# AutomationLabs-sh/AutomationLabsModelPredictiveControl.jl

Measured on AMD Instinct MI355X. Metric: MPC steps/s (batch=4096, nx=12, nu=4, N=30), higher is better.
Workload: dtype f64; 1 GPU; configs[1]: hover-linearised quadrotor nx=12 nu=4 N=30, 4096 instances per GPU, shared model, x0 amplitude classes 0.3/1.0/3.0 interleaved, cold start every step; batch_per_gpu=4096, global_batch=4096, seed=0x5eed0002, setup_ramp_steps=300, admm_max_iter=6, check_every=6, polish=1, warm_state_kept=False, parallelism=instances sharded over 1 GPU(s), 16-instance tile per workgroup

## Files before the change

### automationlabsmodelpredictivecontrol.jl_amd/_capi.py

```python
from __future__ import annotations

import ctypes
import os

import numpy as np

_HERE = os.path.dirname(os.path.abspath(__file__))
LIB_PATH = os.environ.get("ALMPC_LIB") or os.path.join(_HERE, "lib", "libalmpc.so")

ALMPC_OK = 0
ERR_NAMES = {0: "ALMPC_OK", -1: "ALMPC_ERR_INVALID", -2: "ALMPC_ERR_NO_DEVICE", -3: "ALMPC_ERR_HIP",
             -4: "ALMPC_ERR_UNSUPPORTED", -5: "ALMPC_ERR_NOT_DESIGNED", -6: "ALMPC_ERR_NUMERIC"}
FLAG_TIMING = 0x1
FLAG_STRUCTURED = 0x2
SOLVED, MAX_ITER, NON_FINITE, INFEASIBLE = 0, 1, 2, 3


class AlmpcError(RuntimeError):
    def __init__(self, code, msg=""):
        self.code = code
        super().__init__(f"{ERR_NAMES.get(code, code)}: {msg}")


class almpc_opts(ctypes.Structure):
# ... 175 lines not shown
    L.almpc_group_sqp_fnn_state_multipliers.argtypes = [_hp, _dp]
    L.almpc_group_sqp_fnn_solve.argtypes = [_hp, ctypes.c_int, ctypes.c_double, ctypes.POINTER(almpc_opts), _ip, _ip, _dp]
    L.almpc_group_x0_staging.argtypes = [_hp, ctypes.POINTER(_dp)]
    L.almpc_group_update_initialization_staged.argtypes = [_hp, ctypes.POINTER(_dp)]
    L.almpc_group_get_results_async.argtypes = [_hp, ctypes.c_uint32]
    L.almpc_group_get_results_wait.argtypes = [_hp, ctypes.c_int, _dp, _dp, _dp, _dp, _dp, _ip, _ip, _ip]
    for nm_ in ("almpc_group_set_terminal_equality", "almpc_group_set_rho_profile", "almpc_group_set_structured_fallback", "almpc_group_set_state_box",
                "almpc_group_design_batched", "almpc_group_relin_fnn_setup", "almpc_group_relin_fnn_step", "almpc_group_relin_fnn_step_async",
                "almpc_group_relin_fnn_advance", "almpc_group_advance_plant", "almpc_group_sqp_fnn_set_structured", "almpc_group_sqp_fnn_set_step_rule",
                "almpc_group_sqp_fnn_setup", "almpc_group_relin_densenet_setup", "almpc_group_sqp_densenet_setup", "almpc_group_sqp_fnn_start", "almpc_group_sqp_fnn_iterate", "almpc_group_sqp_fnn_skipped", "almpc_group_sqp_fnn_solve", "almpc_group_sqp_fnn_set_hessian",
                "almpc_group_sqp_fnn_set_row_multipliers", "almpc_group_sqp_fnn_state_multipliers",
                "almpc_group_x0_staging", "almpc_group_update_initialization_staged", "almpc_group_get_results_async", "almpc_group_get_results_wait"):
        getattr(L, nm_).restype = ctypes.c_int
    L.almpc_set_start_from.argtypes = [_hp, _hp]
    L.almpc_set_start_from.restype = ctypes.c_int
    L.almpc_timing_samples.argtypes = [_hp, ctypes.c_int, ctypes.POINTER(ctypes.c_int), _fp, _fp, _fp, _fp]
    L.almpc_timing_samples.restype = ctypes.c_int
    for name in ("almpc_x0_staging", "almpc_update_initialization_async", "almpc_get_results_async", "almpc_get_results_wait", "almpc_host_results",
                 "almpc_get_first_input", "almpc_group_create", "almpc_group_size", "almpc_group_shard", "almpc_group_design_shared",
                 "almpc_group_set_reference", "almpc_group_update_initialization", "almpc_group_calculate",
                 "almpc_group_calculate_async", "almpc_group_synchronize", "almpc_group_get_results"):
        getattr(L, name).restype = ctypes.c_int
    for name in ("almpc_create", "almpc_design_shared", "almpc_set_reference", "almpc_update_initialization",
                 "almpc_update_initialization_device", "almpc_calculate", "almpc_calculate_async", "almpc_synchronize",
                 "almpc_get_results", "almpc_get_design", "almpc_device_results", "almpc_get_timing", "almpc_timing_reset",
                 "almpc_timing_summary"):
        getattr(L, name).restype = ctypes.c_int
    _lib = L
    return L


OPT_NO_WARM_STATE = 0x1
OPT_FULL_FIRST_PRODUCT = 0x2
WANT = {"x": 0x01, "e_x": 0x02, "u": 0x04, "e_u": 0x08, "status": 0x10, "iters": 0x20, "polish_iters": 0x40, "u0": 0x80}
SENS = {"K0": 0x1, "dU": 0x2, "dX": 0x4}


def _sens_mask(want):
    mask = 0
    for k in ((want,) if isinstance(want, str) else want):
        if k not in SENS:
            raise ValueError(f"unknown sensitivity {k!r} (one of {sorted(SENS)})")
        mask |= SENS[k]
    if not mask:
        raise ValueError("sensitivity: nothing asked for")
    return mask


def _sens_read(get, handle, check, want, b, n, m, N):
    mask = _sens_mask(want)
    K0 = np.empty((b, n, m)) if mask & SENS["K0"] else None
    dU = np.empty((b, n, N, m)) if mask & SENS["dU"] else None
    dX = np.empty((b, n, N + 1, n)) if mask & SENS["dX"] else None
    rows = np.empty(b, dtype=np.int32)
    check(get(handle, _ptr(K0), _ptr(dU), _ptr(dX), rows.ctypes.data_as(_ip)))
    out = {"rows": rows}
    if K0 is not None: out["K0"] = K0.transpose(0, 2, 1)
    if dU is not None: out["dU"] = dU.transpose(0, 3, 2, 1)
    if dX is not None: out["dX"] = dX.transpose(0, 3, 2, 1)
    return out


def _sens_vjp(call, handle, check, g_u, g_x, act_tol, b, n, m, N):
    g_u = np.ascontiguousarray(np.asarray(g_u, dtype=np.float64).reshape(b, m, N).transpose(0, 2, 1))
    if g_x is not None:
        g_x = np.ascontiguousarray(np.asarray(g_x, dtype=np.float64).reshape(b, n, N + 1).transpose(0, 2, 1))
# ... 924 lines not shown
```

### automationlabsmodelpredictivecontrol.jl_amd/csrc/almpc_api.hip

```cpp
#include "almpc_kernels.hip.h"
#include "almpc_design.hip.h"
#include "almpc_polish_gen.hip.h"
#include "almpc_fnn.hip.h"
#include "almpc_instance.hip.h"
#include "almpc_sqp.hip.h"
#include "almpc_comm.hip.h"
#include "almpc_riccati.hip.h"
#include "almpc_sdual.hip.h"
#include "almpc_dare.hip.h"
#include "almpc_c2d.hip.h"
#include "almpc_sens.hip.h"
#include "almpc_host_math.h"
#include "almpc_switches.h"
#include "almpc_devbuf.h"
#include "../../include/almpc.h"

#ifndef ALMPC_UNITY
#define ALMPC_KERNEL_INSTANCE(...) extern template __global__ __VA_ARGS__;
#include "instances/sdual_a.inc"
#include "instances/sdual_b.inc"
#include "instances/sdual_c.inc"
#include "instances/polish_gen.inc"
#include "instances/step.inc"
#include "instances/instance.inc"
// ... 2255 lines not shown
    HIP_TRY(h, h->dOverflow.once((size_t)h->batch * 33 + 2));
    HIP_TRY(h, hipMemsetAsync(h->dOverflow, 0, 2 * sizeof(int32_t), h->stream));
    HIP_TRY(h, h->dOvfSinv.once((size_t)h->batch * (32 * 32 + 32)));
    gp.ovf = h->dOverflow; gp.ovf_ws = h->dOverflow + 2 + h->batch; gp.ovf_sinv = h->dOvfSinv;
    if (s.lazy_redo) { gp.unsolved = h->redo.dUnsolved; gp.redo_gate = h->redo.dGate; gp.step_serial = h->redo.step_serial; }
    if (h->fallback && !h->ltv && h->sd.ready && !h->sd.sqp && !h->sw.no_redo_start) {
        HIP_TRY(h, h->sd.start_ws.once((size_t)h->batch * 64));
        gp.redo_ws = h->sd.start_ws; gp.redo_sp = h->sd.NT + h->sd.MC; gp.redo_nt = h->sd.NT;
        h->sd.start_ws_fresh = true;
    }
    if (h->s0_basis_ok && !h->batched && !h->ltv && h->fS_stride == 0) gp.s0_basis = h->dS0Basis;
    if (s.mode.rows.mu && sq) { gp.rows = s.mode.rows; gp.rows_map = h->dRowMap; }
    switch (h->np_pairs) {
        case 1: HIP_TRY(h, launch_polish_gen<1>(h, gp)); break;
        case 2: HIP_TRY(h, launch_polish_gen<2>(h, gp)); break;
        case 3: HIP_TRY(h, launch_polish_gen<3>(h, gp)); break;
        default: HIP_TRY(h, launch_polish_gen<4>(h, gp)); break;
    }
    HIP_TRY(h, s.t.mark(2));
    return ALMPC_OK;
}

template <int KS>
hipError_t launch_step_fused(const AdmmParams& ap, const PolishParams& pp, size_t lds, hipStream_t st) {
    const hipError_t e = ensure_dyn_lds(reinterpret_cast<const void*>(k_step_fused<8, KS>), lds);
    if (e != hipSuccess) return e;
    hipLaunchKernelGGL((k_step_fused<8, KS>), dim3(pp.ntiles), dim3(512), lds, st, ap, pp);
    return hipGetLastError();
}

int step_fused_shared(Step& s, const PolishLayout& L) {
    almpc_handle* h = s.h;
    const AdmmParams ap = admm_params(h, s.o, s.keep_state);
    const PolishParams pp = polish_params(s, L);
    HIP_TRY(h, s.t.mark(1));
    HIP_TRY(h, h->ks == 30 ? launch_step_fused<30>(ap, pp, L.l_step, h->stream) : launch_step_fused<32>(ap, pp, L.l_step, h->stream));
    HIP_TRY(h, s.t.mark(2));
    return ALMPC_OK;
}

template <int NZC>
hipError_t launch_step_inst_wave_t(const almpc_handle* h, const AdmmInstParams& ip, const PolishParams& pp, size_t lds) {
    const hipError_t e = ensure_dyn_lds(reinterpret_cast<const void*>(k_step_inst_wave<NZC>), lds);
    if (e != hipSuccess) return e;
    hipLaunchKernelGGL((k_step_inst_wave<NZC>), dim3((unsigned)h->batch), dim3(64), lds, h->stream, ip, pp);
    return hipGetLastError();
}

int step_wave(Step& s, const PolishLayout& L, bool shared) {
    almpc_handle* h = s.h;
    if (shared) HIP_TRY(h, s.t.start());
    const AdmmInstParams ip = admm_inst_params(h, s.o, shared);
    PolishParams pp = polish_params(s, L);
    if (shared) { pp.yflags = nullptr; pp.yflag_words = 0; }
    const size_t wave = (size_t)L.per_wave + (shared ? 0 : (size_t)h->nz * h->nzs);
    const size_t lds = ((size_t)L.SL.total + wave) * sizeof(double);
    pp.sg_off = -1; pp.g_off = shared ? 0 : L.per_wave;
    pp.lds_per_wave = (int)wave;
    pp.direct = 1;
    HIP_TRY(h, s.t.mark(1));
    if (h->nzs <= 16) HIP_TRY(h, launch_step_inst_wave_t<16>(h, ip, pp, lds));
    else if (h->nzs <= 32) HIP_TRY(h, launch_step_inst_wave_t<32>(h, ip, pp, lds));
    else if (h->nzs <= 48) HIP_TRY(h, launch_step_inst_wave_t<48>(h, ip, pp, lds));
    else HIP_TRY(h, launch_step_inst_wave_t<64>(h, ip, pp, lds));
    HIP_TRY(h, s.t.mark(2));
    return ALMPC_OK;
}
// ... 1678 lines not shown
```

### automationlabsmodelpredictivecontrol.jl_amd/csrc/almpc_kernels.hip.h

```cpp
#pragma once
#include <hip/hip_runtime.h>
#include <stdint.h>

#include <map>
#include <mutex>
#include <utility>
#include <type_traits>

namespace almpc {

inline hipError_t ensure_dyn_lds(const void* fn, size_t bytes) {
    if (bytes <= 64 * 1024) return hipSuccess;
    static std::mutex mu;
    static std::map<std::pair<int, const void*>, size_t> cur;
    int dev = 0;
    hipError_t e = hipGetDevice(&dev);
    if (e != hipSuccess) return e;
    std::lock_guard<std::mutex> lock(mu);
    size_t& c = cur[std::make_pair(dev, fn)];
    if (c >= bytes) return hipSuccess;
    e = hipFuncSetAttribute(fn, hipFuncAttributeMaxDynamicSharedMemorySize, (int)bytes);
    if (e == hipSuccess) c = bytes;
    return e;
}
// ... 62 lines not shown
    const double* VFrag;
    const double* v0S;
    long v0S_stride;
    const double* Wp = nullptr;
    const double* rowc = nullptr;
    const double* HFrag;
    const double* FFrag;
    int ksf;
    const double* dvec;
    const double* rhovec;
    const double* umin;
    const double* umax;
    const double* uref;
    long uref_stride;
    const double* xref;
    long xref_stride;
    const double* fS;
    long fS_stride;
    const double* x0;
    double* xs;
    double* zs;
    double* ys;
    double* v0;
    int32_t* status;
    int32_t* iters;
    int32_t* piters;
    int32_t* perm;
    double rho, sigma, alpha, eps_abs, eps_rel;
    int max_iter, check_every, warm;
    int keep_state;
    uint32_t* yflags;
};

template <int NRB, int KS, typename AfterRequests>
__device__ __forceinline__ void admm_body(const AdmmParams& p, double* smem, AfterRequests after_requests) {
    constexpr int RP = 16 * NRB;
    static_assert(4 * KS <= RP, "K padding must fit the row padding");
    double* rhs0 = smem;
    double* rhs1 = smem + RP * TILE;
    double* red = smem + 2 * RP * TILE;
    double* e0s = red + NRB * 8 * TILE;

    const int wv = threadIdx.x >> 6, lane = threadIdx.x & 63;
    const int col = lane & 15, q = lane >> 4;
    const int inst = blockIdx.x * TILE + col;
    const bool valid = inst < p.batch;
    const int instc = valid ? inst : p.batch - 1;
    ALMPC_STAMP(blockIdx.x * NRB + wv, 0);

    constexpr int KSF_FAST = 4;
    const bool tabled = p.rowc != nullptr;
    const bool affine = !p.warm && tabled && p.Wp != nullptr;
    double af[KSF_FAST], aw[KSF_FAST], av[KSF_FAST];
#pragma unroll
    for (int ks = 0; ks < KSF_FAST; ++ks) {
        const bool on = ks < p.ksf;
        const size_t o = ((size_t)(wv * p.ksf + ks)) * 64 + lane;
        af[ks] = on ? p.FFrag[o] : 0.0;
        aw[ks] = (on && affine && 4 * ks + q < p.n) ? p.Wp[(size_t)(4 * ks + q) * p.nzs + wv * 16 + col] : 0.0;
        av[ks] = on ? p.VFrag[o] : 0.0;
    }
    int row[4];
    double dv[4], dinv[4], lo[4], hi[4], fs[4], rho[4], v0s[4], ws[4];
#pragma unroll
    for (int i = 0; i < 4; ++i) row[i] = wv * 16 + q + 4 * i;
    if (tabled) {
#pragma unroll
        for (int i = 0; i < 4; ++i) {
// ... 175 lines not shown
                r[0 * TILE] = m_rp; r[1 * TILE] = m_x; r[2 * TILE] = m_z; r[3 * TILE] = m_rd;
                r[4 * TILE] = m_hx; r[5 * TILE] = m_y; r[6 * TILE] = m_bad;
            }
        }
        __syncthreads();
        if (check) {
            double rp = 0, nx = 0, nzn = 0, rd = 0, nhx = 0, ny = 0, bad = 0;
#pragma unroll 4
            for (int w2 = 0; w2 < NRB; ++w2) {
                const double* r = red + w2 * 8 * TILE + col;
                rp = fmax(rp, r[0 * TILE]); nx = fmax(nx, r[1 * TILE]); nzn = fmax(nzn, r[2 * TILE]);
                rd = fmax(rd, r[3 * TILE]); nhx = fmax(nhx, r[4 * TILE]); ny = fmax(ny, r[5 * TILE]);
                bad = fmax(bad, r[6 * TILE]);
            }
            if (active) {
                const bool conv = (rp <= p.eps_abs + p.eps_rel * fmax(nx, nzn)) &&
                                  (rd <= p.eps_abs + p.eps_rel * fmax(fmax(nhx, ny), nf));
                if (bad > 0.0) { active = false; my_iters = it; my_status = 2; }
                else if (conv) { active = false; my_iters = it; my_status = 0; }
            }
            const bool any_active = __any(active);
            __syncthreads();
            if (!any_active) { double* t = cur; cur = nxt; nxt = t; break; }
        }
        double* t = cur; cur = nxt; nxt = t;
    }

    ALMPC_STAMP(blockIdx.x * NRB + wv, 2);
    if (valid && wv == 0 && q == 0) {
        p.iters[inst] = my_iters;
        p.status[inst] = my_status;
        p.piters[inst] = 0;
    }
    {
        int cntf = 0;
#pragma unroll
        for (int i = 0; i < 4; ++i) cntf += (row[i] < p.nz && yt[i] != 0.0) ? 1 : 0;
        cntf += __shfl_xor(cntf, 16);
        cntf += __shfl_xor(cntf, 32);
        if (q == 0) red[(wv * 8 + 0) * TILE + col] = (double)cntf;
    }
    __syncthreads();
    if (wv == 0 && q == 0) {
        int k0 = valid ? 0 : -1;
        if (valid)
            for (int w2 = 0; w2 < NRB; ++w2) k0 += (int)red[(w2 * 8 + 0) * TILE + col];
        red[(0 * 8 + 1) * TILE + col] = (double)k0;
        __builtin_amdgcn_fence(__ATOMIC_RELEASE, "wavefront");
        __builtin_amdgcn_wave_barrier();
        __builtin_amdgcn_fence(__ATOMIC_ACQUIRE, "wavefront");
        int rank = 0;
        for (int c2 = 0; c2 < TILE; ++c2) {
            const int ko = (int)red[(0 * 8 + 1) * TILE + c2];
            rank += (ko > k0 || (ko == k0 && c2 < col)) ? 1 : 0;
        }
        p.perm[blockIdx.x * TILE + rank] = valid ? inst : -1;
    }
    ALMPC_STAMP(blockIdx.x * NRB + wv, 3);

    constexpr int TS = RP + 2;
    static_assert(TILE * TS <= 2 * RP * TILE, "staging tile must fit the two rhs buffers");
    double* stage = smem;
    auto flush = [&](const double (&v)[4], double* dst) {
        __syncthreads();
#pragma unroll
        for (int i = 0; i < 4; ++i) stage[col * TS + row[i]] = v[i];
        __syncthreads();
        for (int e = 2 * threadIdx.x; e < TILE * RP; e += 2 * blockDim.x) {
            const int ci = e / RP, r = e % RP;
            const int ii = blockIdx.x * TILE + ci;
            if (ii < p.batch)
                *reinterpret_cast<d2v*>(dst + (size_t)ii * p.nzs + r) = *reinterpret_cast<const d2v*>(stage + ci * TS + r);
        }
    };
    const double v0r[4] = {v04[0], v04[1], v04[2], v04[3]};
    double y[4];
#pragma unroll
    for (int i = 0; i < 4; ++i) y[i] = rho[i] * yt[i];
    if (p.keep_state) {
        flush(x, p.xs);
        flush(y, p.ys);
    } else {
        uint32_t mk = 0;
#pragma unroll
        for (int i = 0; i < 4; ++i) {
            const uint32_t b = (uint32_t)(q + 4 * i);
            mk |= (yt[i] < 0.0 ? 1u : 0u) << b;
            mk |= (yt[i] > 0.0 ? 1u : 0u) << (16u + b);
        }
        mk |= (uint32_t)__shfl_xor((int)mk, 16);
        mk |= (uint32_t)__shfl_xor((int)mk, 32);
        if (q == 0 && valid) p.yflags[(size_t)inst * NRB + wv] = mk;
    }
    flush(z, p.zs);
    flush(v0r, p.v0);
    ALMPC_STAMP(blockIdx.x * NRB + wv, 4);
}

template <int NRB, int KS>
__global__ __launch_bounds__(64 * NRB) void k_admm(AdmmParams p) {
    extern __shared__ __attribute__((aligned(16))) double smem[];
    admm_body<NRB, KS>(p, smem, []() {});
}

struct RolloutParams {
    int n, m, N, batch, nzs;
    const double* A;
    const double* B;
    long A_stride = 0, B_stride = 0, d_stride = 0;
    const double* dvec;
    const double* w;
    const double* x0;
    const double* xref;
    long xref_stride;
    const double* uref;
    long uref_stride;
    const double* umin;
    const double* umax;
    double* x;
    double* ex;
    double* u;
    double* eu;
};

struct PolishParams {
    int nz, m, batch, nzs;
    const double* G;
    const double* dvec;
    const double* umin;
    const double* umax;
    const double* uref;
    long uref_stride;
    const double* zs;
    const double* ys;
    const uint32_t* yflags;
    int yflag_words;
    const double* v0;
    double* w;
    int32_t* status;
    int32_t* piters;
    double* sglobal;
    const int32_t* start_rows = nullptr;
    const int32_t* perm;
    int ntiles;
    int lds_per_wave;
    long G_stride, d_stride, A_stride, B_stride;
    int wave_const_off;
    int sg_off;
    int sg_shared_off;
    int g_off;
    int max_iter;
    const int* dflag = nullptr;
    int* unsolved = nullptr;
    int* redo_gate = nullptr;
    int step_serial = 0;
    int direct = 0;
    int fuse_rollout;
    int roll_g, roll_cpl;
    const double* rollM;
    int roll_s, roll_nb;
    RolloutParams roll;
};

__device__ __forceinline__ double readlane_d(double v, int l) {
    int lo = __builtin_amdgcn_readlane(__double2loint(v), l);
    int hi = __builtin_amdgcn_readlane(__double2hiint(v), l);
    return __hiloint2double(hi, lo);
}

__device__ __forceinline__ double fast_rcp_d(double v) {
    double r = __builtin_amdgcn_rcp(v);
    r = __builtin_fma(__builtin_fma(-v, r, 1.0), r, r);
    r = __builtin_fma(__builtin_fma(-v, r, 1.0), r, r);
    return r;
}

typedef double gj16_row[16];
template <int JJ>
__device__ __forceinline__ void gj16_pivot(gj16_row& r, const double (&pj)[16], const double col, const double d, const bool own, const int k,
                                           const int lane) {
    const double invd = fast_rcp_d(d);
    const bool piv = lane == k;
    const double f = piv ? -invd : col * invd;
    const double keep = piv ? 0.0 : 1.0;
#pragma unroll
    for (int jj = 0; jj < 16; ++jj) r[jj] = __builtin_fma(-f, pj[jj], keep * r[jj]);
    if (own) r[JJ] = f;
}

// ... 182 lines not shown
        prev = ev;
        src0 = (s - 1) * n;
        upart(b + 1, acc);
        if (xref_lds) asm volatile("" : "+v"(xr));
        if (ok) {
            gex[t] = ev;
            if (gx) gx[t] = ev + xr;
        }
    }
}

constexpr int POLISH_WAVES = 4;
#ifndef ALMPC_EXP_POLISH_WAVES
#define ALMPC_EXP_POLISH_WAVES 8
#endif
constexpr int POLISH_WAVES_GLDS = ALMPC_EXP_POLISH_WAVES;
constexpr int POLISH_LDS_MIN_PER_WAVE = 128 + 64 + 64 + 32;
struct PolishShared {
    int off_d, off_umin, off_umax, off_uref, off_ab, off_xref, total;
};
__host__ __device__ inline PolishShared polish_shared_layout(int n, int m, int N, int nz, int nzs, int fused) {
    PolishShared L;
    L.off_d = 0;
    L.off_umin = nzs;
    L.off_umax = L.off_umin + m;
    L.off_uref = L.off_umax + m;
    L.off_ab = L.off_uref + nz;
    L.off_xref = L.off_ab + ((fused && fused != 3) ? n * (n + m) : 0);
    L.total = (L.off_xref + (fused ? (N + 1) * n : 0) + 1) & ~1;
    return L;
}
constexpr int POLISH_GLB_PER_INST = 64 * 64;
constexpr int POLISH_SG_SHARED_CAP = 48;

typedef double d2 __attribute__((ext_vector_type(2)));

template <bool GLDS, bool GPRE, int KOFF, bool SGL = false, bool START = false>
__device__ __forceinline__ void polish_body(const PolishParams& p_arg, double* smem) {
    const PolishParams& p = p_arg;
    constexpr int CH = (GLDS || SGL) ? 8 : 16;
    constexpr int NWV = GLDS ? POLISH_WAVES_GLDS : (SGL ? 1 : POLISH_WAVES);
    const int wv = __builtin_amdgcn_readfirstlane(threadIdx.x >> 6), lane_k = threadIdx.x & 63;
    const int nz = p.nz, nzs = p.nzs;
    const double* Gp = p.G;
    const int gs = GLDS ? ((nz + 1) & ~1) : nzs;
    const PolishShared SL = polish_shared_layout(p.roll.n, p.m, p.roll.N, nz, nzs, p.fuse_rollout);
    double* shc = smem + (GLDS ? (size_t)nz * gs : 0);
    double* wave_lds = shc + SL.total + (size_t)wv * p.lds_per_wave;
    int* qcnt = nullptr;
    const bool uref_sh = p.uref_stride == 0, xref_sh = p.roll.xref_stride == 0;
    const bool per_inst = p.G_stride != 0;
    double* cd = shc + SL.off_d;
    double* cab = shc + SL.off_ab;
    if (per_inst) { cd = wave_lds + p.wave_const_off; cab = cd + nzs; }
    {
        constexpr int TPB = 64 * NWV;
        const int n = p.roll.n, m = p.m, N = p.roll.N;
        if (!per_inst)
            for (int t = threadIdx.x; t < nzs; t += TPB) shc[SL.off_d + t] = p.dvec[t];
        for (int t = threadIdx.x; t < m; t += TPB) { shc[SL.off_umin + t] = p.umin[t]; shc[SL.off_umax + t] = p.umax[t]; }
        if (uref_sh)
            for (int t = threadIdx.x; t < nz; t += TPB) shc[SL.off_uref + t] = p.uref[t];
        if (p.fuse_rollout) {
            if (!per_inst && p.fuse_rollout != 3) {
                for (int t = threadIdx.x; t < n * n; t += TPB) shc[SL.off_ab + t] = p.roll.A[t];
                for (int t = threadIdx.x; t < n * m; t += TPB) shc[SL.off_ab + n * n + t] = p.roll.B[t];
            }
            if (xref_sh)
                for (int t = threadIdx.x; t < (N + 1) * n; t += TPB) shc[SL.off_xref + t] = p.roll.xref[t];
        }
    }
    ALMPC_STAMP(8192 + blockIdx.x * 8 + wv, 0);
    if constexpr (GLDS && !GPRE) {
        const int hs = gs / 2;
        const bool lane_in = lane_k < hs;
        const int lq = lane_in ? lane_k : 0;
        for (int r0_ = wv; r0_ < nz; r0_ += POLISH_WAVES_GLDS * 8) {
            d2 v[8];
#pragma unroll
            for (int u = 0; u < 8; ++u) {
                const int r = r0_ + u * POLISH_WAVES_GLDS;
                v[u] = *reinterpret_cast<const d2*>(p.G + (size_t)(r < nz ? r : 0) * nzs + 2 * lq);
            }
#pragma unroll
            for (int u = 0; u < 8; ++u) {
                const int r = r0_ + u * POLISH_WAVES_GLDS;
                if (r < nz && lane_in) *reinterpret_cast<d2*>(smem + (size_t)r * gs + 2 * lq) = v[u];
            }
        }
    }
    if constexpr (GLDS) {
        qcnt = reinterpret_cast<int*>(shc + SL.total + (size_t)POLISH_WAVES_GLDS * p.lds_per_wave);
        if (threadIdx.x == 0) { qcnt[0] = POLISH_WAVES_GLDS; qcnt[1] = -1; }
        Gp = smem;
    }
    __syncthreads();
  auto process = [&](const int inst) {
    auto ka_ = __builtin_amdgcn_kernarg_segment_ptr();
    asm volatile("" : "+s"(ka_));
    const PolishParams& p = *(const PolishParams*)((const char*)ka_ + KOFF);
    int lane = lane_k;
    asm volatile("" : "+v"(lane));
    ALMPC_STAMP(inst, 8);
    if constexpr (!GLDS) {
        if (per_inst) {
            if constexpr (SGL) {
                double* gl = wave_lds + p.g_off;
                const char* src = reinterpret_cast<const char*>(GL(p.G) + (size_t)inst * p.G_stride) + lane * 16;
                if (lane < nzs / 2)
                    for (int r = 0; r < nz; ++r)
                        __builtin_amdgcn_global_load_lds((const __attribute__((address_space(1))) void*)(src + (size_t)r * nzs * 8),
                                                         (__attribute__((address_space(3))) void*)(gl + (size_t)r * nzs), 16, 0, 0);
                Gp = gl;
            } else
            Gp = GL(p.G) + (size_t)inst * p.G_stride;
            const int n_ = p.roll.n, m_ = p.m;
            for (int t = lane; t < nzs; t += 64) cd[t] = GL(p.dvec)[(size_t)inst * p.d_stride + t];
            if (p.fuse_rollout) {
                for (int t = lane; t < n_ * n_; t += 64) cab[t] = GL(p.roll.A)[(size_t)inst * p.A_stride + t];
                for (int t = lane; t < n_ * m_; t += 64) cab[n_ * n_ + t] = GL(p.roll.B)[(size_t)inst * p.B_stride + t];
            }
            if constexpr (SGL) __builtin_amdgcn_s_waitcnt(0);
            wave_fence_lds();
        }
    }
    const int st_in = GL(p.status)[inst];
    const size_t base = (size_t)inst * nzs;
    const int r0 = 2 * lane, r1 = 2 * lane + 1;
    const bool in0 = r0 < nz, in1 = r1 < nz;
    const bool inrow = r0 < nzs;
    const int rc = inrow ? r0 : 0;
    const bool skip = (st_in == 2);

    double* rowbuf = wave_lds;
    double* pbufa = rowbuf + 128;
    double* pbufb = pbufa + 64;
    int* wrow_s = reinterpret_cast<int*>(pbufb + 64);
    double* Sg;
    int cap2 = 64;
    bool own_slot = false;
    const bool sg_lds = SGL && p.sg_off >= 0;
    if (sg_lds) Sg = wave_lds + p.sg_off;
    else Sg = GL(p.sglobal) + (size_t)inst * POLISH_GLB_PER_INST;

    double lo0 = 0, hi0 = 0, lo1 = 0, hi1 = 0, v00, v01, w0 = 0, w1 = 0, y0, y1, z0, z1;
    double x0r = 0.0;
    if (p.fuse_rollout && lane < p.roll.n) x0r = GL(p.roll.x0)[(size_t)inst * p.roll.n + lane];
    {
        const d2 dv = *reinterpret_cast<const d2*>(cd + rc);
        const d2 vv = *reinterpret_cast<const d2*>(GL(p.v0) + base + rc);
        d2 yy;
        if (p.yflags) {
            const uint32_t wd = GL(p.yflags)[(size_t)inst * p.yflag_words + (rc >> 4)];
            const uint32_t b = (uint32_t)(rc & 15);
            yy[0] = (double)(int)((wd >> (16u + b)) & 1u) - (double)(int)((wd >> b) & 1u);
            yy[1] = (double)(int)((wd >> (17u + b)) & 1u) - (double)(int)((wd >> (b + 1u)) & 1u);
        } else {
            yy = *reinterpret_cast<const d2*>(GL(p.ys) + base + rc);
        }
        const d2 zz = *reinterpret_cast<const d2*>(GL(p.zs) + base + rc);
        v00 = vv[0]; v01 = vv[1]; y0 = yy[0]; y1 = yy[1]; z0 = zz[0]; z1 = zz[1];
        double urp0, urp1;
        if (uref_sh) {
            urp0 = shc[SL.off_uref + (in0 ? r0 : 0)]; urp1 = shc[SL.off_uref + (in1 ? r1 : 0)];
            asm volatile("" : "+v"(urp0), "+v"(urp1));
        } else {
            const double* ug = GL(p.uref) + (size_t)inst * p.uref_stride;
            urp0 = ug[in0 ? r0 : 0]; urp1 = ug[in1 ? r1 : 0];
        }
        if (in0) {
            const double di = 1.0 / dv[0], ur = urp0;
            lo0 = (shc[SL.off_umin + r0 % p.m] - ur) * di; hi0 = (shc[SL.off_umax + r0 % p.m] - ur) * di; w0 = fmin(fmax(z0, lo0), hi0);
        } else { v00 = 0.0; y0 = 0.0; z0 = 0.0; }
        if (in1) {
            const double di = 1.0 / dv[1], ur = urp1;
            lo1 = (shc[SL.off_umin + r1 % p.m] - ur) * di; hi1 = (shc[SL.off_umax + r1 % p.m] - ur) * di; w1 = fmin(fmax(z1, lo1), hi1);
        } else { v01 = 0.0; y1 = 0.0; z1 = 0.0; }
    }
    int wrow = 0, wsd = 0;
    double wbnd = 0.0;
    double lam = 0.0;
    bool act0 = false, act1 = false;
    double bnd0 = 0.0, bnd1 = 0.0;
    double t0 = v00, t1 = v01;
    int k = 0;
    bool overflow = false;
    ALMPC_ACC_DECL
    wrow_s[lane] = 0;
    const int hpos = lane & 31, hhf = lane >> 5;
    double Sr[16];
#pragma unroll
    for (int t = 0; t < 16; ++t) Sr[t] = 0.0;
    auto bcast16 = [&](const double* buf, double (&o)[16]) {
// ... 297 lines not shown
                if (r1 == jmin) w1 = bval;
                ALMPC_ACC(5);
                add_row(m, jmin, bval, sd);
                fresh = false;
                continue;
            }
            if (!act0) w0 = t0;
            if (!act1) w1 = t1;
            bool ok = true;
            int vi = 0;
            if (k > 0) {
                const bool mine = lowhalf && pos < k;
                const double viol = mine ? ((wsd > 0) ? -lam : lam) : -__builtin_inf();
                const double lmax = wave_max(mine ? fabs(lam) : 0.0);
                const double vmax = wave_max(viol);
                ok = vmax <= 1e-12 * fmax(1.0, lmax);
                vi = __builtin_ctzll(__ballot(mine && viol == vmax));
            }
            if (ok) {
                if (fresh) { fin = 0; return; }
                recompute(m);
                fresh = true;
                --it;
                continue;
            }
            remove_pos(m, vi);
            fresh = false;
        }
    };
    auto tier2_home = [&](int need) {
        if constexpr (GLDS) {
            if (p.sg_shared_off >= 0 && need <= POLISH_SG_SHARED_CAP) {
                int got = 0;
                if (lane == 0) got = (atomicCAS(qcnt + 1, -1, wv) == -1) ? 1 : 0;
                got = __builtin_amdgcn_readfirstlane(got);
                if (got) { own_slot = true; cap2 = POLISH_SG_SHARED_CAP; Sg = shc + p.sg_shared_off; }
            }
        }
    };
    auto slot_to_global = [&]() {
        double* Gs = GL(p.sglobal) + (size_t)inst * POLISH_GLB_PER_INST;
        for (int c = 0; c < POLISH_SG_SHARED_CAP; c += 8) {
            double v[8];
#pragma unroll
            for (int t = 0; t < 8; ++t) v[t] = Sg[(c + t) * 64 + lane];
#pragma unroll
            for (int t = 0; t < 8; ++t) Gs[(c + t) * 64 + lane] = v[t];
        }
        for (int c = POLISH_SG_SHARED_CAP; c < 64; ++c) Gs[c * 64 + lane] = (c == lane) ? 1.0 : 0.0;
        __builtin_amdgcn_fence(__ATOMIC_RELEASE, "workgroup");
        __builtin_amdgcn_wave_barrier();
        __builtin_amdgcn_fence(__ATOMIC_ACQUIRE, "workgroup");
        if (lane == 0) atomicExch(qcnt + 1, -1);
        own_slot = false; cap2 = 64; Sg = Gs;
    };
    auto to_global = [&]() {
#pragma unroll
        for (int t = 0; t < 16; ++t) {
            Sg[(16 * hhf + t) * 64 + hpos] = Sr[t];
            Sg[(16 * hhf + t) * 64 + 32 + hpos] = 0.0;
        }
#pragma unroll 4
        for (int c = 32; c < cap2; ++c) Sg[c * 64 + lane] = 0.0;
        if (lane >= 32 && lane < cap2) Sg[lane * 64 + lane] = 1.0;
        if (lane >= 32) lam = 0.0;
        sync_s(PolishMode<true>{});
    };
// ... 297 lines not shown
                const int t = t0 + 64 * u + lane;
                tt[u] = t < nx ? t : nx - 1;
                const int kq = (int)(((float)tt[u] + 0.5f) * inv_n);
                ev[u] = Z[(size_t)tt[u] + (size_t)kq * m];
            }
            if (xref_sh) {
#pragma unroll
                for (int u = 0; u < 4; ++u) xr[u] = shc[SL.off_xref + tt[u]];
                asm volatile("" : "+v"(xr[0]), "+v"(xr[1]), "+v"(xr[2]), "+v"(xr[3]));
            } else {
                const double* xg = GL(rp.xref) + (size_t)inst * rp.xref_stride;
#pragma unroll
                for (int u = 0; u < 4; ++u) xr[u] = xg[tt[u]];
            }
#pragma unroll
            for (int u = 0; u < 4; ++u) {
                const int t = t0 + 64 * u + lane;
                if (t < nx) {
                    GL(rp.ex)[xo + t] = ev[u];
                    GL(rp.x)[xo + t] = (t < n) ? x0r : ev[u] + xr[u];
                }
            }
        }
        ALMPC_STAMP(inst, 14);
    }
  };

    if constexpr (GLDS) {
        ALMPC_STAMP(8192 + blockIdx.x * 8 + wv, 1);
        [[maybe_unused]] int nproc = 0;
        for (int i = wv;;) {
            const int tile = (i >> 4) * (int)gridDim.x + (int)blockIdx.x;
            if (tile >= p.ntiles) break;
            const int inst = p.perm[tile * 16 + (i & 15)];
            if (inst >= 0) {
                process(inst);
                ++nproc;
            }
            if (lane_k == 0) i = atomicAdd(qcnt, 1);
            i = __builtin_amdgcn_readfirstlane(i);
        }
        ALMPC_STAMP(8192 + blockIdx.x * 8 + wv, 2);
#ifdef ALMPC_STAMPS
        if (g_stamps && (threadIdx.x & 63) == 0) g_stamps[(size_t)(8192 + blockIdx.x * 8 + wv) * 16 + 3] = nproc;
#endif
    } else {
        const int slot = blockIdx.x * NWV + wv;
        if (p.direct) {
            if (slot < p.batch) process(slot);
        } else if (slot < p.ntiles * 16) {
            const int inst = p.perm[(slot % p.ntiles) * 16 + slot / p.ntiles];
            if (inst >= 0) process(inst);
        }
    }
}

template <bool GLDS>
__global__ __launch_bounds__(64 * (GLDS ? POLISH_WAVES_GLDS : POLISH_WAVES))
__attribute__((amdgpu_waves_per_eu(GLDS ? POLISH_WAVES_GLDS / 4 : 2, GLDS ? POLISH_WAVES_GLDS / 4 : 2)))
void k_polish(PolishParams p_arg) {
    extern __shared__ __attribute__((aligned(16))) double smem[];
    polish_body<GLDS, false, 0>(p_arg, smem);
}

template <int START = 0>
__global__ __launch_bounds__(64) void k_polish_sgl(PolishParams p_arg) {
    extern __shared__ __attribute__((aligned(16))) double smem[];
    polish_body<false, false, 0, true, START != 0>(p_arg, smem);
}

constexpr int STEP_KOFF = (int)((sizeof(AdmmParams) + 7) & ~size_t(7));

template <int NRB, int KS>
__global__ __launch_bounds__(64 * NRB) __attribute__((amdgpu_waves_per_eu(2, 2)))
void k_step_fused(AdmmParams ap, PolishParams pp) {
    extern __shared__ __attribute__((aligned(16))) double smem[];
    if constexpr (NRB != POLISH_WAVES_GLDS) return;
    const int wv = __builtin_amdgcn_readfirstlane(threadIdx.x >> 6), lane = threadIdx.x & 63;
    const int gs = (pp.nz + 1) & ~1, hs = gs / 2;
    auto request_g = [&]() __attribute__((always_inline)) {
        for (int r = wv; r < pp.nz; r += NRB) {
            if (lane < hs) {
                const char* src = reinterpret_cast<const char*>(pp.G + (size_t)r * pp.nzs) + lane * 16;
                __builtin_amdgcn_global_load_lds((const __attribute__((address_space(1))) void*)src,
                                                 (__attribute__((address_space(3))) void*)(smem + (size_t)r * gs), 16, 0, 0);
            }
        }
    };
    admm_body<NRB, KS>(ap, smem + (size_t)pp.nz * gs, request_g);
    __builtin_amdgcn_s_waitcnt(0);
    __syncthreads();
    polish_body<true, true, STEP_KOFF>(pp, smem);
}


template <int WAVES>
__global__ __launch_bounds__(64 * WAVES) void k_rollout(RolloutParams p) {
    extern __shared__ __attribute__((aligned(16))) double smem[];
    const int n = p.n, m = p.m, N = p.N;
    const int nz = m * N, nx = n * (N + 1);
    double* As = smem;
    double* Bs = As + n * n;
    double* wbuf = Bs + n * m;
    ALMPC_STAMP(blockIdx.x * WAVES + (threadIdx.x >> 6), 4);
    const double* Ag = p.A + (size_t)blockIdx.x * WAVES * p.A_stride;
    const double* Bg = p.B + (size_t)blockIdx.x * WAVES * p.B_stride;
    for (int t = threadIdx.x; t < n * n; t += blockDim.x) As[t] = Ag[t];
    for (int t = threadIdx.x; t < n * m; t += blockDim.x) Bs[t] = Bg[t];
    __syncthreads();
    const int wv = threadIdx.x >> 6, lane = threadIdx.x & 63;
    const int inst = blockIdx.x * WAVES + wv;
    if (inst >= p.batch) return;
    ALMPC_STAMP(inst, 0);
    double* e = wbuf + (size_t)wv * (nx + nz);
    double* v = e + nx;
    for (int r = lane; r < nz; r += 64) {
        const double ur = p.uref[(size_t)inst * p.uref_stride + r];
        const double uu = fmin(fmax(p.w[(size_t)inst * p.nzs + r] * p.dvec[(size_t)inst * p.d_stride + r] + ur, p.umin[r % m]), p.umax[r % m]);
        const double ev = uu - ur;
        v[r] = ev;
        p.eu[(size_t)inst * nz + r] = ev;
        p.u[(size_t)inst * nz + r] = uu;
// ... 70 lines not shown
```

### include/almpc.h

```cpp
#ifndef ALMPC_H
#define ALMPC_H

#include <stdint.h>

#ifdef __cplusplus
extern "C" {
#endif

#define ALMPC_VERSION_MAJOR 0
#define ALMPC_VERSION_MINOR 1

typedef struct almpc_handle almpc_handle;

typedef enum almpc_status {
    ALMPC_OK = 0,
    ALMPC_ERR_INVALID = -1,
    ALMPC_ERR_NO_DEVICE = -2,
    ALMPC_ERR_HIP = -3,
    ALMPC_ERR_UNSUPPORTED = -4,
    ALMPC_ERR_NOT_DESIGNED = -5,
    ALMPC_ERR_NUMERIC = -6
} almpc_status;

typedef enum almpc_solve_status {
    ALMPC_SOLVED = 0,
    ALMPC_MAX_ITER = 1,
    ALMPC_NON_FINITE = 2,
    ALMPC_INFEASIBLE = 3
} almpc_solve_status;

typedef struct almpc_opts {
    double rho;
    double sigma;
    double alpha;
    double eps_abs;
    double eps_rel;
    int32_t max_iter;
    int32_t check_every;
    int32_t polish;
    int32_t polish_max_iter;
    int32_t warm_start;
    int32_t reserved[3];
} almpc_opts;

#define ALMPC_OPT_NO_WARM_STATE 0x1
#define ALMPC_OPT_FULL_FIRST_PRODUCT 0x2

void almpc_default_opts(almpc_opts* opts);

#define ALMPC_FLAG_TIMING 0x1u
#define ALMPC_FLAG_STRUCTURED 0x2u

int almpc_create(almpc_handle** out, int n, int m, int N, int batch, int device_id, uint32_t flags);
void almpc_destroy(almpc_handle* h);
const char* almpc_last_error(const almpc_handle* h);

int almpc_set_terminal_equality(almpc_handle* h, int on);

int almpc_set_rho_profile(almpc_handle* h, int mode);

int almpc_set_step_fusion(almpc_handle* h, int on);

int almpc_set_structured_fallback(almpc_handle* h, int on);

int almpc_set_start_from(almpc_handle* h, almpc_handle* src);

int almpc_set_state_box(almpc_handle* h, const double* xmin, const double* xmax);

int almpc_design_shared(almpc_handle* h, const double* A, const double* B, const double* Q,
                        const double* R, const double* S, const double* P, const double* umin,
                        const double* umax, const double* xmin, const double* xmax, double rho,
                        double sigma);

int almpc_design_batched(almpc_handle* h, const double* A_batch, const double* B_batch, const double* Q,
                         const double* R, const double* S, const double* P, int P_per_instance,
                         const double* umin, const double* umax, double rho, double sigma);

int almpc_design_ltv(almpc_handle* h, const double* A_all, const double* B_all, const double* c_all, const double* xbar,
                     const double* ubar, const double* xref, const double* uref, const double* Q, const double* R,
// ... 207 lines not shown
```

Baseline: 17590 batch-steps/s (one step = 4096 instance QP solves).

## Hand off ADMM state to polish through LDS records instead of HBM

In the fused step kernel, the ADMM phase now writes each instance's z, v0, sign mask, status and instance id into per-rank LDS records (wave slots plus the shared second-tier slot) and preloads polish constants. The polish phase then reads from these records instead of round-tripping through global zs/v0/yflags/status and perm. This removes HBM writes and reads between the two phases and the redundant constant reload. It adds an atomic counter so the shared slot is not claimed by a polish wave before staged records are consumed. It keeps an opt-out flag for the old HBM path.

```diff
diff --git a/automationlabsmodelpredictivecontrol.jl_amd/_capi.py b/automationlabsmodelpredictivecontrol.jl_amd/_capi.py
--- a/automationlabsmodelpredictivecontrol.jl_amd/_capi.py
+++ b/automationlabsmodelpredictivecontrol.jl_amd/_capi.py
@@ -231,6 +231,7 @@
 
 OPT_NO_WARM_STATE = 0x1
 OPT_FULL_FIRST_PRODUCT = 0x2
+OPT_HBM_HANDOFF = 0x4
 WANT = {"x": 0x01, "e_x": 0x02, "u": 0x04, "e_u": 0x08, "status": 0x10, "iters": 0x20, "polish_iters": 0x40, "u0": 0x80}
 SENS = {"K0": 0x1, "dU": 0x2, "dX": 0x4}
 
diff --git a/automationlabsmodelpredictivecontrol.jl_amd/csrc/almpc_api.hip b/automationlabsmodelpredictivecontrol.jl_amd/csrc/almpc_api.hip
--- a/automationlabsmodelpredictivecontrol.jl_amd/csrc/almpc_api.hip
+++ b/automationlabsmodelpredictivecontrol.jl_amd/csrc/almpc_api.hip
@@ -2311,7 +2311,8 @@
 int step_fused_shared(Step& s, const PolishLayout& L) {
     almpc_handle* h = s.h;
     const AdmmParams ap = admm_params(h, s.o, s.keep_state);
-    const PolishParams pp = polish_params(s, L);
+    PolishParams pp = polish_params(s, L);
+    pp.handoff = (!s.keep_state && L.sg_shared_off >= 0 && !(s.o.reserved[0] & ALMPC_OPT_HBM_HANDOFF)) ? 1 : 0;
     HIP_TRY(h, s.t.mark(1));
     HIP_TRY(h, h->ks == 30 ? launch_step_fused<30>(ap, pp, L.l_step, h->stream) : launch_step_fused<32>(ap, pp, L.l_step, h->stream));
     HIP_TRY(h, s.t.mark(2));
diff --git a/automationlabsmodelpredictivecontrol.jl_amd/csrc/almpc_kernels.hip.h b/automationlabsmodelpredictivecontrol.jl_amd/csrc/almpc_kernels.hip.h
--- a/automationlabsmodelpredictivecontrol.jl_amd/csrc/almpc_kernels.hip.h
+++ b/automationlabsmodelpredictivecontrol.jl_amd/csrc/almpc_kernels.hip.h
@@ -118,8 +118,17 @@
     uint32_t* yflags;
 };
 
-template <int NRB, int KS, typename AfterRequests>
-__device__ __forceinline__ void admm_body(const AdmmParams& p, double* smem, AfterRequests after_requests) {
+__device__ __forceinline__ void lds_barrier();
+
+constexpr int HANDOFF_STATUS = 8, HANDOFF_INST = 9;
+__device__ __forceinline__ int handoff_rot(int rank) { return 4 * (rank & 7); }
+
+struct NoHandoff {
+    static constexpr bool possible = false;
+};
+
+template <int NRB, int KS, typename AfterRequests, typename Hand>
+__device__ __forceinline__ void admm_body(const AdmmParams& p, double* smem, AfterRequests after_requests, const Hand& hand) {
     constexpr int RP = 16 * NRB;
     static_assert(4 * KS <= RP, "K padding must fit the row padding");
     double* rhs0 = smem;
@@ -361,14 +370,67 @@
         p.status[inst] = my_status;
         p.piters[inst] = 0;
     }
-    {
+    auto count_guess = [&]() {
         int cntf = 0;
 #pragma unroll
         for (int i = 0; i < 4; ++i) cntf += (row[i] < p.nz && yt[i] != 0.0) ? 1 : 0;
         cntf += __shfl_xor(cntf, 16);
         cntf += __shfl_xor(cntf, 32);
         if (q == 0) red[(wv * 8 + 0) * TILE + col] = (double)cntf;
-    }
+    };
+    auto sign_word = [&]() -> uint32_t {
+        uint32_t mk = 0;
+#pragma unroll
+        for (int i = 0; i < 4; ++i) {
+            const uint32_t b = (uint32_t)(q + 4 * i);
+            mk |= (yt[i] < 0.0 ? 1u : 0u) << b;
+            mk |= (yt[i] > 0.0 ? 1u : 0u) << (16u + b);
+        }
+        mk |= (uint32_t)__shfl_xor((int)mk, 16);
+        mk |= (uint32_t)__shfl_xor((int)mk, 32);
+        return mk;
+    };
+    if constexpr (Hand::possible) {
+        if (hand.on) {
+            static_assert(RP == 128, "a hand-off record holds 128 rows of z and of v0");
+            constexpr int TPB = 64 * NRB;
+            const double hc0 = hand.load_const((int)threadIdx.x), hc1 = hand.load_const((int)threadIdx.x + TPB);
+            count_guess();
+            lds_barrier();
+            int k0 = valid ? 0 : -1;
+            if (valid)
+                for (int w2 = 0; w2 < NRB; ++w2) k0 += (int)red[(w2 * 8 + 0) * TILE + col];
+            const int key = k0 * 16 + (15 - col);
+            int rank = 0;
+#pragma unroll
+            for (int c2 = 0; c2 < TILE; ++c2) rank += (__builtin_amdgcn_readlane(key, c2) > key) ? 1 : 0;
+            if (wv == 0 && q == 0) p.perm[blockIdx.x * TILE + rank] = valid ? inst : -1;
+            const uint32_t mk = sign_word();
+            ALMPC_STAMP(blockIdx.x * NRB + wv, 3);
+            lds_barrier();
+            double* rec = hand.record(rank);
+            const int rot = handoff_rot(rank);
+#pragma unroll
+            for (int i = 0; i < 4; ++i) {
+                const int o = (row[i] + rot) & (RP - 1);
+                rec[o] = z[i];
+                rec[RP + o] = v04[i];
+            }
+            int* ri = reinterpret_cast<int*>(rec + 2 * RP);
+            if (q == 0) ri[wv] = (int)mk;
+            if (wv == 0 && q == 0) { ri[HANDOFF_STATUS] = my_status; ri[HANDOFF_INST] = valid ? inst : -1; }
+            hand.store_const((int)threadIdx.x, hc0);
+            hand.store_const((int)threadIdx.x + TPB, hc1);
+            for (int t = (int)threadIdx.x + 2 * TPB; t < hand.SL.total; t += TPB) hand.store_const(t, hand.load_const(t));
+            if (threadIdx.x == 0) {
+                const int nvalid = p.batch - (int)blockIdx.x * TILE;
+                hand.init_queue(nvalid > NRB ? (nvalid < TILE ? nvalid : TILE) - NRB : 0);
+            }
+            ALMPC_STAMP(blockIdx.x * NRB + wv, 4);
+            return;
+        }
+    }
+    count_guess();
     __syncthreads();
     if (wv == 0 && q == 0) {
         int k0 = valid ? 0 : -1;
@@ -410,15 +472,7 @@
         flush(x, p.xs);
         flush(y, p.ys);
     } else {
-        uint32_t mk = 0;
-#pragma unroll
-        for (int i = 0; i < 4; ++i) {
-            const uint32_t b = (uint32_t)(q + 4 * i);
-            mk |= (yt[i] < 0.0 ? 1u : 0u) << b;
-            mk |= (yt[i] > 0.0 ? 1u : 0u) << (16u + b);
-        }
-        mk |= (uint32_t)__shfl_xor((int)mk, 16);
-        mk |= (uint32_t)__shfl_xor((int)mk, 32);
+        const uint32_t mk = sign_word();
         if (q == 0 && valid) p.yflags[(size_t)inst * NRB + wv] = mk;
     }
     flush(z, p.zs);
@@ -429,7 +483,7 @@
 template <int NRB, int KS>
 __global__ __launch_bounds__(64 * NRB) void k_admm(AdmmParams p) {
     extern __shared__ __attribute__((aligned(16))) double smem[];
-    admm_body<NRB, KS>(p, smem, []() {});
+    admm_body<NRB, KS>(p, smem, []() {}, NoHandoff{});
 }
 
 struct RolloutParams {
@@ -484,6 +538,7 @@
     int* redo_gate = nullptr;
     int step_serial = 0;
     int direct = 0;
+    int handoff = 0;
     int fuse_rollout;
     int roll_g, roll_cpl;
     const double* rollM;
@@ -732,6 +787,8 @@
 }
 constexpr int POLISH_GLB_PER_INST = 64 * 64;
 constexpr int POLISH_SG_SHARED_CAP = 48;
+constexpr int HANDOFF_REC = POLISH_LDS_MIN_PER_WAVE;
+static_assert((TILE - 8) * HANDOFF_REC <= POLISH_SG_SHARED_CAP * 64, "the records of ranks 8..15 must fit the second-tier slot");
 
 typedef double d2 __attribute__((ext_vector_type(2)));
 
@@ -753,7 +810,9 @@
     double* cd = shc + SL.off_d;
     double* cab = shc + SL.off_ab;
     if (per_inst) { cd = wave_lds + p.wave_const_off; cab = cd + nzs; }
-    {
+    bool handed = false;
+    if constexpr (GLDS && GPRE) handed = p.handoff != 0;
+    if (!handed) {
         constexpr int TPB = 64 * NWV;
         const int n = p.roll.n, m = p.m, N = p.roll.N;
         if (!per_inst)
@@ -791,11 +850,11 @@
     }
     if constexpr (GLDS) {
         qcnt = reinterpret_cast<int*>(shc + SL.total + (size_t)POLISH_WAVES_GLDS * p.lds_per_wave);
-        if (threadIdx.x == 0) { qcnt[0] = POLISH_WAVES_GLDS; qcnt[1] = -1; }
+        if (!handed && threadIdx.x == 0) { qcnt[0] = POLISH_WAVES_GLDS; qcnt[1] = -1; qcnt[2] = 0; }
         Gp = smem;
     }
-    __syncthreads();
-  auto process = [&](const int inst) {
+    if (!handed) __syncthreads();
+  auto process = [&](const int inst, const double* rec, const int rank) {
     auto ka_ = __builtin_amdgcn_kernarg_segment_ptr();
     asm volatile("" : "+s"(ka_));
     const PolishParams& p = *(const PolishParams*)((const char*)ka_ + KOFF);
@@ -824,7 +883,11 @@
             wave_fence_lds();
         }
     }
-    const int st_in = GL(p.status)[inst];
+    bool from_rec = false;
+    if constexpr (GLDS && GPRE) from_rec = rec != nullptr;
+    int st_in;
+    if (from_rec) st_in = __builtin_amdgcn_readfirstlane(reinterpret_cast<const int*>(rec + 256)[HANDOFF_STATUS]);
+    else st_in = GL(p.status)[inst];
     const size_t base = (size_t)inst * nzs;
     const int r0 = 2 * lane, r1 = 2 * lane + 1;
     const bool in0 = r0 < nz, in1 = r1 < nz;
@@ -848,8 +911,22 @@
     if (p.fuse_rollout && lane < p.roll.n) x0r = GL(p.roll.x0)[(size_t)inst * p.roll.n + lane];
     {
         const d2 dv = *reinterpret_cast<const d2*>(cd + rc);
-        const d2 vv = *reinterpret_cast<const d2*>(GL(p.v0) + base + rc);
-        d2 yy;
+        d2 vv, yy, zz;
+        if (from_rec) {
+            const int o = (rc + handoff_rot(rank)) & 127;
+            zz = *reinterpret_cast<const d2*>(rec + o);
+            vv = *reinterpret_cast<const d2*>(rec + 128 + o);
+            uint32_t wd = (uint32_t)reinterpret_cast<const int*>(rec + 256)[rc >> 4];
+            asm volatile("" : "+v"(zz), "+v"(vv), "+v"(wd));
+            const uint32_t b = (uint32_t)(rc & 15);
+            yy[0] = (double)(int)((wd >> (16u + b)) & 1u) - (double)(int)((wd >> b) & 1u);
+            yy[1] = (double)(int)((wd >> (17u + b)) & 1u) - (double)(int)((wd >> (b + 1u)) & 1u);
+            if (rank >= POLISH_WAVES_GLDS) {
+                __builtin_amdgcn_fence(__ATOMIC_RELEASE, "workgroup");
+                if (lane == 0) atomicSub(qcnt + 2, 1);
+            }
+        } else {
+        vv = *reinterpret_cast<const d2*>(GL(p.v0) + base + rc);
         if (p.yflags) {
             const uint32_t wd = GL(p.yflags)[(size_t)inst * p.yflag_words + (rc >> 4)];
             const uint32_t b = (uint32_t)(rc & 15);
@@ -858,7 +935,8 @@
         } else {
             yy = *reinterpret_cast<const d2*>(GL(p.ys) + base + rc);
         }
-        const d2 zz = *reinterpret_cast<const d2*>(GL(p.zs) + base + rc);
+        zz = *reinterpret_cast<const d2*>(GL(p.zs) + base + rc);
+        }
         v00 = vv[0]; v01 = vv[1]; y0 = yy[0]; y1 = yy[1]; z0 = zz[0]; z1 = zz[1];
         double urp0, urp1;
         if (uref_sh) {
@@ -1222,7 +1300,8 @@
         if constexpr (GLDS) {
             if (p.sg_shared_off >= 0 && need <= POLISH_SG_SHARED_CAP) {
                 int got = 0;
-                if (lane == 0) got = (atomicCAS(qcnt + 1, -1, wv) == -1) ? 1 : 0;
+                if (lane == 0)
+                    got = (__hip_atomic_load(qcnt + 2, __ATOMIC_RELAXED, __HIP_MEMORY_SCOPE_WORKGROUP) == 0 && atomicCAS(qcnt + 1, -1, wv) == -1) ? 1 : 0;
                 got = __builtin_amdgcn_readfirstlane(got);
                 if (got) { own_slot = true; cap2 = POLISH_SG_SHARED_CAP; Sg = shc + p.sg_shared_off; }
             }
@@ -1586,9 +1665,17 @@
         for (int i = wv;;) {
             const int tile = (i >> 4) * (int)gridDim.x + (int)blockIdx.x;
             if (tile >= p.ntiles) break;
-            const int inst = p.perm[tile * 16 + (i & 15)];
+            int inst;
+            const double* rec = nullptr;
+            if (handed) {
+                if (i >= p.batch - (int)blockIdx.x * TILE) break;
+                rec = i < POLISH_WAVES_GLDS ? wave_lds : shc + p.sg_shared_off + (size_t)(i - POLISH_WAVES_GLDS) * HANDOFF_REC;
+                inst = __builtin_amdgcn_readfirstlane(reinterpret_cast<const int*>(rec + 256)[HANDOFF_INST]);
+            } else {
+                inst = p.perm[tile * 16 + (i & 15)];
+            }
             if (inst >= 0) {
-                process(inst);
+                process(inst, rec, i);
                 ++nproc;
             }
             if (lane_k == 0) i = atomicAdd(qcnt, 1);
@@ -1601,10 +1688,10 @@
     } else {
         const int slot = blockIdx.x * NWV + wv;
         if (p.direct) {
-            if (slot < p.batch) process(slot);
+            if (slot < p.batch) process(slot, nullptr, 0);
         } else if (slot < p.ntiles * 16) {
             const int inst = p.perm[(slot % p.ntiles) * 16 + slot / p.ntiles];
-            if (inst >= 0) process(inst);
+            if (inst >= 0) process(inst, nullptr, 0);
         }
     }
 }
@@ -1624,6 +1711,34 @@
 }
 
 constexpr int STEP_KOFF = (int)((sizeof(AdmmParams) + 7) & ~size_t(7));
+
+struct StepHandoff {
+    static constexpr bool possible = true;
+    const PolishParams& pp;
+    double* shc;
+    PolishShared SL;
+    bool on;
+    __device__ __forceinline__ double* record(int rank) const {
+        return rank < POLISH_WAVES_GLDS ? shc + SL.total + (size_t)rank * pp.lds_per_wave
+                                        : shc + pp.sg_shared_off + (size_t)(rank - POLISH_WAVES_GLDS) * HANDOFF_REC;
+    }
+    __device__ __forceinline__ double load_const(int t) const {
+        const int n = pp.roll.n, nx = (pp.roll.N + 1) * n;
+        double v = 0.0;
+        if (t < SL.off_umin) v = GL(pp.dvec)[t];
+        else if (t < SL.off_umax) v = GL(pp.umin)[t - SL.off_umin];
+        else if (t < SL.off_uref) v = GL(pp.umax)[t - SL.off_umax];
+        else if (t < SL.off_ab) { if (pp.uref_stride == 0) v = GL(pp.uref)[t - SL.off_uref]; }
+        else if (t < SL.off_xref) { const int u = t - SL.off_ab; v = u < n * n ? GL(pp.roll.A)[u] : GL(pp.roll.B)[u - n * n]; }
+        else if (pp.fuse_rollout && pp.roll.xref_stride == 0 && t < SL.off_xref + nx) v = GL(pp.roll.xref)[t - SL.off_xref];
+        return v;
+    }
+    __device__ __forceinline__ void store_const(int t, double v) const { if (t < SL.total) shc[t] = v; }
+    __device__ __forceinline__ void init_queue(int staged) const {
+        int* qcnt = reinterpret_cast<int*>(shc + SL.total + (size_t)POLISH_WAVES_GLDS * pp.lds_per_wave);
+        qcnt[0] = POLISH_WAVES_GLDS; qcnt[1] = -1; qcnt[2] = staged;
+    }
+};
 
 template <int NRB, int KS>
 __global__ __launch_bounds__(64 * NRB) __attribute__((amdgpu_waves_per_eu(2, 2)))
@@ -1641,7 +1756,9 @@
             }
         }
     };
-    admm_body<NRB, KS>(ap, smem + (size_t)pp.nz * gs, request_g);
+    double* un = smem + (size_t)pp.nz * gs;
+    const StepHandoff hand{pp, un, polish_shared_layout(pp.roll.n, pp.m, pp.roll.N, pp.nz, pp.nzs, pp.fuse_rollout), pp.handoff != 0};
+    admm_body<NRB, KS>(ap, un, request_g, hand);
     __builtin_amdgcn_s_waitcnt(0);
     __syncthreads();
     polish_body<true, true, STEP_KOFF>(pp, smem);
diff --git a/include/almpc.h b/include/almpc.h
--- a/include/almpc.h
+++ b/include/almpc.h
@@ -45,6 +45,7 @@
 
 #define ALMPC_OPT_NO_WARM_STATE 0x1
 #define ALMPC_OPT_FULL_FIRST_PRODUCT 0x2
+#define ALMPC_OPT_HBM_HANDOFF 0x4
 
 void almpc_default_opts(almpc_opts* opts);
 
```

New measurement: 17890 batch-steps/s (one step = 4096 instance QP solves) (median of 6 runs). +1.7%, better.
